# omarkhursheed/whisper-sae

Measured on AMD Instinct MI355X. Metric: activations/sec through SAE train step (d=384->3072, k=32), higher is better.
Workload: dtype bf16; 1 GPU; BASELINE.json configs[1]: TopKSAE 384->3072 k=32 train step, synthetic activations resident in the HBM ring buffer; batch_per_gpu=16384, global_batch=16384, ring_rows_per_gpu=4194304, parallelism=dp1

## Files before the change

whisper-sae_amd/csrc/wsae_common.h:

```cpp
#pragma once

#include <hip/hip_runtime.h>
#include <stdint.h>
#include <stdio.h>

#include "wsae.h"

void wsae_set_error(const char* fmt, ...);

#define WSAE_HIP_CHECK(expr)                                                              \
    do {                                                                                  \
        hipError_t e_ = (expr);                                                           \
        if (e_ != hipSuccess) {                                                           \
            wsae_set_error("%s failed: %s (%s:%d)", #expr, hipGetErrorString(e_), __FILE__, \
                           __LINE__);                                                     \
            return WSAE_ERR_HIP;                                                          \
        }                                                                                 \
    } while (0)

#define WSAE_REQUIRE(cond, ...)          \
    do {                                 \
        if (!(cond)) {                   \
            wsae_set_error(__VA_ARGS__); \
            return WSAE_ERR_INVALID;     \
        }                                \
    } while (0)

#define WSAE_LAUNCH_CHECK()                                                                  \
    do {                                                                                     \
        hipError_t e_ = hipGetLastError();                                                   \
        if (e_ != hipSuccess) {                                                              \
            wsae_set_error("kernel launch failed: %s (%s:%d)", hipGetErrorString(e_), __FILE__, \
                           __LINE__);                                                        \
            return WSAE_ERR_HIP;                                                             \
        }                                                                                    \
    } while (0)

typedef __bf16 bf16_t;
typedef __bf16 bf16x8 __attribute__((ext_vector_type(8)));
typedef __bf16 bf16x4 __attribute__((ext_vector_type(4)));
typedef float f32x16 __attribute__((ext_vector_type(16)));
typedef float f32x4 __attribute__((ext_vector_type(4)));
typedef float f32x2 __attribute__((ext_vector_type(2)));
typedef __bf16 bf16x2 __attribute__((ext_vector_type(2)));

static inline int64_t ceil_div64(int64_t a, int64_t b) { return (a + b - 1) / b; }
static inline int ceil_div(int a, int b) { return (a + b - 1) / b; }

#define WSAE_MAX_PARTIALS 1024
#define WSAE_WGRAD_MAX_SPLIT 8

struct wsae_prof {
    unsigned mask;
    int max_samples;
    int count[WSAE_K_COUNT];
    hipEvent_t* ev[WSAE_K_COUNT];
};

struct wsae_ctx {
    wsae_prof prof;
    int D, H, K, maxB, prec, device;
    const float* relu_l1w;
    int loss_cols;
    int cus;
    int comm_reserve;
    int64_t P;
    int64_t off[5];
    bf16_t* We_bf16;
    bf16_t* WdT_bf16;
    float* c_fold;
    void* xb;
    void* xT;
    void* gT;
    float* g;
    bf16_t* gb;
    int g_is_bf16;
    int xT_valid;
    int g32_valid;
    float* pre;
    float* smax;
    int smax_valid;
    uint32_t* tmin;
    int tmin_cur;
    int strip_predict;
    float tg_fixed_s;
    int pred_valid;
    const void* pred_x;
    const int32_t* pred_rows;
    float* part_loss;
    float* part_l0;
    float* part_dbd;
    float* part_sq;
    float* colnorm;
    float* wg_slabs;
    float* dbe_slab;
    float* dbpre_part;
    uint32_t* ent_pos;
    void* ent_hid;
    void* ent_dpre;
    int32_t* ent_off;
    int ent_valid;
    const float* ent_vals;
    int ent_B;
    const float* wire_dec_vals;
    int wire_dec_B;
    int32_t* counters;
    int32_t* dead_list;
    int32_t* row_order;
    int relu_fp8;
    void* relu_ws;
    int relu_x_B;
    int relu_g_B;
    float* fired;
    const float* wire_metrics;
    int n_dec_blocks;
    int n_sq_parts;
    float* dbd2;
    int32_t* btk_ws;
    int btk_k;
    int btk_mode;
    wsae_batch_topk_state* btk_state;
    size_t ws_bytes;
};

#define WSAE_PROF_BEGIN(ctx, id, st)                                                          \
    const bool prof_on_##id = ((ctx)->prof.mask >> (id)) & 1u &&                               \
                              (ctx)->prof.count[id] < (ctx)->prof.max_samples;                 \
    if (prof_on_##id) (void)hipEventRecord((ctx)->prof.ev[id][2 * (ctx)->prof.count[id]], st)
#define WSAE_PROF_END(ctx, id, st)                                                            \
    if (prof_on_##id) {                                                                       \
        (void)hipEventRecord((ctx)->prof.ev[id][2 * (ctx)->prof.count[id] + 1], st);           \
        (ctx)->prof.count[id]++;                                                              \
    }

#ifdef __HIPCC__

#define WSAE_WAVE 64

template <int M>
__device__ __forceinline__ uint32_t lane_xor_u32(uint32_t x, int lane) {
    if constexpr (M == 1) return (uint32_t)__builtin_amdgcn_update_dpp(0, (int)x, 0xB1, 0xF, 0xF, false);
    else if constexpr (M == 2) return (uint32_t)__builtin_amdgcn_update_dpp(0, (int)x, 0x4E, 0xF, 0xF, false);
    else if constexpr (M == 4) {
        const uint32_t up = (uint32_t)__builtin_amdgcn_update_dpp(0, (int)x, 0x104, 0xF, 0xF, false);
        const uint32_t dn = (uint32_t)__builtin_amdgcn_update_dpp(0, (int)x, 0x114, 0xF, 0xF, false);
        return (lane & 4) ? dn : up;
    } else if constexpr (M == 8) return (uint32_t)__builtin_amdgcn_update_dpp(0, (int)x, 0x128, 0xF, 0xF, false);
    else if constexpr (M == 16) {
        const auto r = __builtin_amdgcn_permlane16_swap((int)x, (int)x, false, false);
        return (uint32_t)((lane & 16) ? r[0] : r[1]);
    } else {
        static_assert(M == 32, "lane_xor_u32: M must be a power of two <= 32");
        const auto r = __builtin_amdgcn_permlane32_swap((int)x, (int)x, false, false);
        return (uint32_t)((lane & 32) ? r[0] : r[1]);
    }
}

__device__ __forceinline__ float wave_sum(float v) {
    const int lane = threadIdx.x & 63;
    v += __uint_as_float(lane_xor_u32<32>(__float_as_uint(v), lane));
    v += __uint_as_float(lane_xor_u32<16>(__float_as_uint(v), lane));
    v += __uint_as_float(lane_xor_u32<8>(__float_as_uint(v), lane));
    v += __uint_as_float(lane_xor_u32<4>(__float_as_uint(v), lane));
    v += __uint_as_float(lane_xor_u32<2>(__float_as_uint(v), lane));
    v += __uint_as_float(lane_xor_u32<1>(__float_as_uint(v), lane));
    return v;
}
__device__ __forceinline__ float wave_max(float v) {
    const int lane = threadIdx.x & 63;
    v = fmaxf(v, __uint_as_float(lane_xor_u32<32>(__float_as_uint(v), lane)));
    v = fmaxf(v, __uint_as_float(lane_xor_u32<16>(__float_as_uint(v), lane)));
    v = fmaxf(v, __uint_as_float(lane_xor_u32<8>(__float_as_uint(v), lane)));
    v = fmaxf(v, __uint_as_float(lane_xor_u32<4>(__float_as_uint(v), lane)));
    v = fmaxf(v, __uint_as_float(lane_xor_u32<2>(__float_as_uint(v), lane)));
    v = fmaxf(v, __uint_as_float(lane_xor_u32<1>(__float_as_uint(v), lane)));
    return v;
}
__device__ __forceinline__ int wave_sum_i(int v) {
    const int lane = threadIdx.x & 63;
    v += (int)lane_xor_u32<32>((uint32_t)v, lane);
    v += (int)lane_xor_u32<16>((uint32_t)v, lane);
    v += (int)lane_xor_u32<8>((uint32_t)v, lane);
    v += (int)lane_xor_u32<4>((uint32_t)v, lane);
    v += (int)lane_xor_u32<2>((uint32_t)v, lane);
    v += (int)lane_xor_u32<1>((uint32_t)v, lane);
    return v;
}

__device__ __forceinline__ float block_sum(float v, float* scratch) {
    v = wave_sum(v);
    const int lane = threadIdx.x & 63, w = threadIdx.x >> 6, nw = blockDim.x >> 6;
    __syncthreads();
    if (lane == 0) scratch[w] = v;
    __syncthreads();
    float r = 0.f;
    if (threadIdx.x == 0)
        for (int i = 0; i < nw; ++i) r += scratch[i];
    return r;
}

#define TICKET_GROUPS 32
#define TICKET_WORDS (1 + TICKET_GROUPS)
__device__ __forceinline__ bool grid_ticket(unsigned long long* t, unsigned payload, unsigned* total) {
    const unsigned nblk = gridDim.x * gridDim.y;
    const unsigned bid = blockIdx.y * gridDim.x + blockIdx.x;
    const unsigned ngrp = nblk < TICKET_GROUPS ? nblk : TICKET_GROUPS;
    const unsigned grp = bid % ngrp;
    const unsigned gsz = (nblk - grp + ngrp - 1) / ngrp;
    const unsigned long long add = (1ull << 32) | payload;
    const unsigned long long o1 = __hip_atomic_fetch_add(t + 1 + grp, add, __ATOMIC_RELAXED, __HIP_MEMORY_SCOPE_AGENT);
    if ((unsigned)(o1 >> 32) != gsz - 1) return false;
    __hip_atomic_store(t + 1 + grp, 0ull, __ATOMIC_RELAXED, __HIP_MEMORY_SCOPE_AGENT);
    const unsigned long long add2 = (1ull << 32) | (unsigned)((o1 + add) & 0xFFFFFFFFull);
    const unsigned long long o2 = __hip_atomic_fetch_add(t, add2, __ATOMIC_RELAXED, __HIP_MEMORY_SCOPE_AGENT);
    if ((unsigned)(o2 >> 32) != ngrp - 1) return false;
    __hip_atomic_store(t, 0ull, __ATOMIC_RELAXED, __HIP_MEMORY_SCOPE_AGENT);
    *total = (unsigned)((o2 + add2) & 0xFFFFFFFFull);
    return true;
}

__device__ __forceinline__ float4 nt_load4(const float4* p) {
    const f32x4 v = __builtin_nontemporal_load((const f32x4*)p);
    return make_float4(v[0], v[1], v[2], v[3]);
}
__device__ __forceinline__ void nt_store4(float4* p, const float4& a) {
    f32x4 v;
    v[0] = a.x; v[1] = a.y; v[2] = a.z; v[3] = a.w;
    __builtin_nontemporal_store(v, (f32x4*)p);
}

template <int DT>
__device__ __forceinline__ float load_act(const void* p, int64_t i) {
    if (DT == WSAE_DT_BF16) return (float)((const bf16_t*)p)[i];
    return ((const float*)p)[i];
}

#endif

int wsae_internal_stage(wsae_ctx* ctx, const float* params, const void* x, int x_dtype, const int32_t* rows, int B, hipStream_t st);
int wsae_internal_stage_rows(wsae_ctx* ctx, const float* params, const void* x, int x_dtype, const int32_t* rows, int B, hipStream_t st);
int wsae_internal_stage_and_gemm(wsae_ctx* ctx, const float* params, const void* x, int x_dtype, const int32_t* rows,
                                 int B, float* pre, int64_t* step_count, int direct, hipStream_t st, bool predicate = false);
int wsae_internal_topk(wsae_ctx* ctx, int B, float* vals, int32_t* idx, int32_t* fb, hipStream_t st);
int wsae_internal_encode_topk(wsae_ctx* ctx, const float* params, const void* x, int x_dtype, const int32_t* rows, int B,
                              float* vals, int32_t* idx, int64_t* step_count, int32_t* fb, hipStream_t st);
bool wsae_internal_strips_ok(const wsae_ctx* ctx);
size_t wsae_internal_batch_topk_ws_bytes();
int wsae_internal_batch_topk(wsae_ctx* ctx, float* vals, int B, int k_batch, int mode, wsae_batch_topk_state* state,
                             hipStream_t st);
bool wsae_internal_decode_mfma_ok(const wsae_ctx* c);
int wsae_internal_decode_mfma(wsae_ctx* c, const float* params, const void* x, int x_dtype, const int32_t* rows,
                              const float* vals, const int32_t* idx, int B, float* recon, int want_bwd, float* dpre,
                              int want_g32, int64_t* last_activated, const int64_t* step_count, wsae_stats* stats,
                              hipStream_t st);
bool wsae_internal_gemm256d_fp8(wsae_ctx* c, const void* A, int64_t lda, const void* Bt, int64_t ldb, const float* rscale,
                                const float* cscale, const float* bias, float* C, int64_t ldc, int M, int N, int K,
                                hipStream_t st);
bool wsae_internal_gemm256d(wsae_ctx* c, const void* A, int64_t lda, const void* Bt, int64_t ldb, const float* bias, float* C,
                            int64_t ldc, int M, int N, int K, int nsplit, int64_t cz, hipStream_t st);

enum { GX_EPI_PLAIN = 0, GX_EPI_RELU = 1, GX_EPI_DPRE = 2 };
struct GxEpi {
    const float* bias;
    float* c;
    int64_t ldc, cz;
    bf16_t* out16;
    uint64_t* bits;
    int64_t ldbits;
    int64_t ld16;
    const float* colw;
    float l1;
    float* part;
    int nslots;
    float* colpart;
    const float* rscale;
    const float* cscale;
    float* rowmax;
};
bool wsae_internal_gemm256x(wsae_ctx* c, int a_rm, int b_rm, int epi, const void* A, int64_t lda, const void* Bm, int64_t ldb,
                            int M, int N, int K, int nsplit, const GxEpi& e, hipStream_t st, int fp8 = 0);
int wsae_internal_relu_wgrad(wsae_ctx* ctx, const void* hid, const void* dpre, const void* xb, const void* gb, int B, float* grads,
                             hipStream_t st);
```

whisper-sae_amd/csrc/wsae_encode.hip:

```cpp
#include "wsae_common.h"
#include "wsae_mfma.h"
#include "wsae_topk.h"

template <typename T>
__device__ __forceinline__ void store4(T* p, const float (&v)[4]) {
    if (sizeof(T) == 2) {
        bf16x4 o;
#pragma unroll
        for (int i = 0; i < 4; ++i) o[i] = (bf16_t)v[i];
        *(bf16x4*)p = o;
    } else {
        *(float4*)p = make_float4(v[0], v[1], v[2], v[3]);
    }
}

template <int XDT>
__device__ __forceinline__ void load4(const void* x, int64_t i, float (&v)[4]) {
    if (XDT == WSAE_DT_BF16) {
        const bf16x4 t = *(const bf16x4*)((const bf16_t*)x + i);
#pragma unroll
        for (int q = 0; q < 4; ++q) v[q] = (float)t[q];
    } else {
        const float4 t = *(const float4*)((const float*)x + i);
        v[0] = t.x; v[1] = t.y; v[2] = t.z; v[3] = t.w;
// ... 263 lines not shown
                        const float rs = rscale[min(b, B - 1)];
                        v.x *= rs * cs4.x; v.y *= rs * cs4.y; v.z *= rs * cs4.z; v.w *= rs * cs4.w;
                    }
                    v.x += bv4.x; v.y += bv4.y; v.z += bv4.z; v.w += bv4.w;
                    if (b < B && hcol < H) *(float4*)(Cz + (int64_t)b * ldp + hcol) = v;
                    if (smax) {
                        float m = fmaxf(fmaxf(v.x, v.y), fmaxf(v.z, v.w));
                        m = fmaxf(m, __int_as_float(__builtin_amdgcn_update_dpp(0, __float_as_int(m), 0xB1, 0xF, 0xF, false)));
                        m = fmaxf(m, __int_as_float(__builtin_amdgcn_update_dpp(0, __float_as_int(m), 0x4E, 0xF, 0xF, false)));
                        if ((lane & 3) == 0 && b < B && hcol < H) smax[(int64_t)b * (H >> 4) + (hcol >> 4)] = m;
                    }
                }
                __builtin_amdgcn_wave_barrier();
            }
        }
#pragma unroll
        for (int j = 0; j < 4; ++j) ar[j] = ar_n[j];
    }
    dma_wait();
#ifdef WSAE_ENC_STAMPS
    if (lane == 0)
        for (int i = 0; i < 8; ++i) atomicAdd(&enc_stamp_sum[i], en_acc[i]);
#endif
}
template <typename T>
__device__ __forceinline__ void slab_load_rows(SlabRegs<T>& r, const T* __restrict__ base, int64_t ld, const int32_t* __restrict__ arows,
                                               int row0, int n_rows, int k0, int k_total, int tid) {
    constexpr int EPC = 16 / (int)sizeof(T);
    auto chunk = [&](int c) -> uint4 {
        const int row = row0 + (c >> 3), k = k0 + (c & 7) * EPC;
        if (row < n_rows && k < k_total) return *(const uint4*)(base + (int64_t)arows[row] * ld + k);
        return make_uint4(0, 0, 0, 0);
    };
    r.v0 = chunk(tid); r.v1 = chunk(tid + 256); r.v2 = chunk(tid + 512); r.v3 = chunk(tid + 768);
}

template <typename T>
__global__ void __launch_bounds__(256)
encode_gemm_kernel(const T* __restrict__ xb, const T* __restrict__ W, const float* __restrict__ bias,
                   float* __restrict__ pre, int ldp, int B, int H, int D, const int32_t* __restrict__ arows,
                   int64_t* __restrict__ step_count) {
    extern __shared__ __attribute__((aligned(16))) char smem[];
    char* As = smem;
    char* Bs = smem + TILE_LDS_BYTES;
    const int tid = threadIdx.x, lane = tid & 63, wave = tid >> 6;
    const int wm = wave >> 1, wn = wave & 1;
    const int m0 = blockIdx.y * TILE_M, n0 = blockIdx.x * TILE_N;
    constexpr int KT = Mfma<T>::KT;
    if (step_count && blockIdx.x == 0 && blockIdx.y == 0 && tid == 0) *step_count += 1;

    f32x16 acc[2][2];
#pragma unroll
    for (int i = 0; i < 2; ++i)
#pragma unroll
        for (int j = 0; j < 2; ++j)
#pragma unroll
            for (int r = 0; r < 16; ++r) acc[i][j][r] = 0.f;

    SlabRegs<T> ra, rb;
    if (arows) slab_load_rows<T>(ra, xb, D, arows, m0, B, 0, D, tid);
    else slab_load<T>(ra, xb, D, m0, B, 0, D, tid);
    slab_load<T>(rb, W, D, n0, H, 0, D, tid);
    const int nk = (D + KT - 1) / KT;
    for (int kt = 0; kt < nk; ++kt) {
        slab_store<T>(ra, As, tid);
        slab_store<T>(rb, Bs, tid);
        __syncthreads();
        if (kt + 1 < nk) {
            if (arows) slab_load_rows<T>(ra, xb, D, arows, m0, B, (kt + 1) * KT, D, tid);
            else slab_load<T>(ra, xb, D, m0, B, (kt + 1) * KT, D, tid);
            slab_load<T>(rb, W, D, n0, H, (kt + 1) * KT, D, tid);
        }
        Mfma<T>::slab(As, Bs, wm * 64, wn * 64, lane, acc);
        __syncthreads();
    }
    const int col = lane & 31, rq = lane >> 5;
#pragma unroll
    for (int mi = 0; mi < 2; ++mi)
#pragma unroll
        for (int ni = 0; ni < 2; ++ni) {
            const int h = n0 + wn * 64 + ni * 32 + col;
            if (h >= H) continue;
            const float bv = bias[h];
#pragma unroll
            for (int r = 0; r < 16; ++r) {
                const int b = m0 + wm * 64 + mi * 32 + (r & 3) + 8 * (r >> 2) + 4 * rq;
                if (b < B) pre[(int64_t)b * ldp + h] = acc[mi][ni][r] + bv;
            }
        }
}

__global__ void __launch_bounds__(256)
encode_direct_kernel(const bf16_t* __restrict__ xa, const int32_t* __restrict__ arows, const bf16_t* __restrict__ W,
                     const float* __restrict__ bias, float* __restrict__ pre, int ldp, int B, int H, int D,
                     int64_t* __restrict__ step_count) {
    const int lane = threadIdx.x & 63, wave = threadIdx.x >> 6;
    if (step_count && blockIdx.x == 0 && blockIdx.y == 0 && threadIdx.x == 0) *step_count += 1;
    const int n0 = blockIdx.x * 32, m0 = blockIdx.y * 128 + wave * 32;
    if (m0 >= B) return;
    const int r = lane & 31, h = lane >> 5;
    const int mrow = min(m0 + r, B - 1);
    const int64_t arow = arows ? (int64_t)arows[mrow] : (int64_t)mrow;
    const bf16_t* ap = xa + arow * D + 8 * h;
    const bf16_t* bp = W + (int64_t)min(n0 + r, H - 1) * D + 8 * h;
    f32x16 acc;
#pragma unroll
    for (int i = 0; i < 16; ++i) acc[i] = 0.f;
    const int nk = D / 16;
    for (int k0 = 0; k0 < nk; k0 += 8) {
        bf16x8 a[8], b[8];
#pragma unroll
        for (int j = 0; j < 8; ++j) {
            const int kk = min(k0 + j, nk - 1);
            a[j] = *(const bf16x8*)(ap + 16 * kk);
            b[j] = *(const bf16x8*)(bp + 16 * kk);
        }
#pragma unroll
        for (int j = 0; j < 8; ++j)
            if (k0 + j < nk) acc = __builtin_amdgcn_mfma_f32_32x32x16_bf16(a[j], b[j], acc, 0, 0, 0);
    }
    const int n = n0 + r;
    if (n >= H) return;
    const float bv = bias[n];
#pragma unroll
    for (int i = 0; i < 16; ++i) {
        const int m = m0 + (i & 3) + 8 * (i >> 2) + 4 * h;
        if (m < B) pre[(int64_t)m * ldp + n] = acc[i] + bv;
    }
}

#define TOPK_CAP 256

__global__ void __launch_bounds__(256) topk_kernel(const float* __restrict__ pre, int B, int H, int K,
                                                   float* __restrict__ vals, int32_t* __restrict__ idx,
                                                   int32_t* __restrict__ fallback_rows) {
    __shared__ uint64_t lists[4][TOPK_CAP];
    const int lane = threadIdx.x & 63, wave = threadIdx.x >> 6;
    const int b = blockIdx.x * 4 + wave;
    if (b >= B) return;
    const float* row = pre + (int64_t)b * H;
    uint64_t* list = lists[wave];
    float* vrow = vals + (int64_t)b * K;
    int32_t* irow = idx + (int64_t)b * K;

    uint64_t kmin = 0;
    if (K <= 64) {
        float m = -INFINITY;
        bool any = false;
        for (int e = lane * 4; e < H; e += 256) {
            const float4 v = *(const float4*)(row + e);
            m = fmaxf(fmaxf(m, fmaxf(v.x, v.y)), fmaxf(v.z, v.w));
            any = true;
        }
        uint64_t mk[1] = {any ? ((uint64_t)f32_ord(m) << 32) : 0ull};
        wave_sort_desc<1>(mk, lane);
        const uint32_t thi = __shfl((uint32_t)(mk[0] >> 32), K - 1, 64);
        kmin = (uint64_t)thi << 32;
    }
    const int count = topk_compact<TOPK_CAP>(row, H, kmin, list, lane);
    if (count > TOPK_CAP || count < K) {
        topk_row_generic<TOPK_CAP>(row, H, K, list, lane, vrow, irow, fallback_rows);
        return;
    }
    topk_emit_any<TOPK_CAP>(list, count, K, lane, vrow, irow);
}

#define TOPK_STRIP 8

template <int VPL>
__global__ void __launch_bounds__(256)
topk_rows_kernel(const float* __restrict__ pre, int B, int H, int K, float* __restrict__ vals,
                 int32_t* __restrict__ idx, int32_t* __restrict__ fallback_rows) {
    __shared__ uint64_t lists[4][TOPK_CAP];
    __shared__ uint64_t strips[4][64 * TOPK_STRIP];
    const int lane = threadIdx.x & 63, wave = threadIdx.x >> 6;
    const int b = blockIdx.x * 4 + wave;
    if (b >= B) return;
    const float* row = pre + (int64_t)b * H;
    uint64_t* list = lists[wave];
    uint64_t* strip = strips[wave] + lane * TOPK_STRIP;

    float4 v[VPL];
    float m = -INFINITY;
#pragma unroll
    for (int i = 0; i < VPL; ++i) {
        const int e = lane * 4 + 256 * i;
        v[i] = e < H ? *(const float4*)(row + e) : make_float4(-INFINITY, -INFINITY, -INFINITY, -INFINITY);
        m = fmaxf(fmaxf(m, fmaxf(v[i].x, v[i].y)), fmaxf(v[i].z, v[i].w));
    }
    uint32_t mk[1] = {f32_ord(m)};
    wave_sort_desc<1, uint32_t>(mk, lane);
    const uint32_t thi = __shfl(mk[0], K - 1, 64);

    int cnt = 0;
#pragma unroll
    for (int i = 0; i < VPL; ++i) {
        const float vv[4] = {v[i].x, v[i].y, v[i].z, v[i].w};
#pragma unroll
        for (int c = 0; c < 4; ++c) {
            const uint32_t o = f32_ord(vv[c]);
            if (o >= thi && lane * 4 + 256 * i + c < H) {
                if (cnt < TOPK_STRIP) strip[cnt] = ((uint64_t)o << 32) | (uint32_t)(~(uint32_t)(lane * 4 + 256 * i + c));
                ++cnt;
            }
        }
    }
    int incl = cnt;
#pragma unroll
    for (int o = 1; o < 64; o <<= 1) {
        const int n = __shfl_up(incl, o, 64);
        if (lane >= o) incl += n;
    }
    const int total = __shfl(incl, 63, 64);
    float* vrow = vals + (int64_t)b * K;
    int32_t* irow = idx + (int64_t)b * K;
    if (__any(cnt > TOPK_STRIP) || total > TOPK_CAP || total < K) {
        topk_row_generic<TOPK_CAP>(row, H, K, list, lane, vrow, irow, fallback_rows);
        return;
    }
    const int off = incl - cnt;
    for (int s_ = 0; s_ < cnt; ++s_) list[off + s_] = strip[s_];
    __builtin_amdgcn_wave_barrier();
    topk_emit_any<TOPK_CAP>(list, total, K, lane, vrow, irow);
}

template <int SPL, int NTOP>
__global__ void __launch_bounds__(256) __attribute__((amdgpu_waves_per_eu(8, 8)))
topk_strips_kernel(const float* pre, const float* __restrict__ smax, int B, int H, int K,
                   float* __restrict__ vals, int32_t* __restrict__ idx, int32_t* __restrict__ fallback_rows, StripFix fix,
                   const uint32_t* tmin) {
    __shared__ uint64_t lists[4][TOPK_CAP];
    __shared__ int strips[4][TS_MAX_STRIPS];
    const int lane = threadIdx.x & 63, wave = threadIdx.x >> 6;
    const int b = blockIdx.x * 4 + wave;
    if (b >= B) return;
    fix.tg = tmin ? *(const float*)(tmin + TG_USED) : -INFINITY;
    topk_strips_row<SPL, NTOP, TOPK_CAP>(pre + (int64_t)b * H, smax + (int64_t)b * (H >> 4), H, K, lane, lists[wave],
                                         strips[wave], vals + (int64_t)b * K, idx + (int64_t)b * K, fallback_rows, nullptr,
                                         nullptr, tmin != nullptr, fix, b);
}

__global__ void __launch_bounds__(256) densify_kernel(const float* __restrict__ vals, const int32_t* __restrict__ idx,
                                                      int B, int H, int K, float* __restrict__ hidden) {
    const int64_t i = (int64_t)blockIdx.x * 256 + threadIdx.x;
    if (i >= (int64_t)B * K) return;
    const int b = (int)(i / K);
    const float v = vals[i];
    hidden[(int64_t)b * H + idx[i]] = v > 0.f ? v : 0.f;
}

static int round_up(int a, int b) { return (a + b - 1) / b * b; }

template <typename T>
static int stage_batch(wsae_ctx* c, const float* params, const void* x, int x_dtype, const int32_t* rows, int B,
                       int64_t* step_count, hipStream_t st, bool want_xT = true) {
    const int D = c->D;
    const int ldT = round_up(B, 128);
    dim3 sg(ceil_div(ldT, 64), ceil_div(D, 64));
    T* xT = want_xT ? (T*)c->xT : nullptr;
    WSAE_PROF_BEGIN(c, WSAE_K_STAGE_BATCH, st);
    if (!want_xT && sizeof(T) == 2 && x_dtype == WSAE_DT_BF16 && D % 8 == 0) {
        const int64_t nchunks = (int64_t)B * (D / 8);
        stage_rows_copy_kernel<<<(unsigned)ceil_div64(nchunks, 512), 256, 0, st>>>((const uint4*)x, rows, (uint4*)c->xb, nchunks, D / 8,
                                                                                 step_count);
    } else if (x_dtype == WSAE_DT_F32)
        stage_batch_kernel<WSAE_DT_F32, T><<<sg, 256, 0, st>>>(x, rows, params + c->off[4], (T*)c->xb, xT, B, D, ldT, step_count);
    else
        stage_batch_kernel<WSAE_DT_BF16, T><<<sg, 256, 0, st>>>(x, rows, params + c->off[4], (T*)c->xb, xT, B, D, ldT, step_count);
    WSAE_PROF_END(c, WSAE_K_STAGE_BATCH, st);
    WSAE_LAUNCH_CHECK();
    return WSAE_OK;
}

template <typename T>
static bool persistent_ok(const wsae_ctx* c, int B) {
    constexpr int KT = SWZ_ROW_BYTES / (int)sizeof(T);
    return B >= 2048 && c->H % 256 == 0 && c->D % (2 * KT) == 0;
}

template <typename T>
static int gemm_dense(wsae_ctx* c, const float* params, int B, float* pre, int ldp, const T* xa, const int32_t* arows,
                      int64_t* step_count, hipStream_t st, bool predicate = false) {
    const T* W = sizeof(T) == 2 ? (const T*)c->We_bf16 : (const T*)(params + c->off[0]);
    const float* bias = sizeof(T) == 2 ? c->c_fold : params + c->off[2];
    const int H = c->H;
    WSAE_PROF_BEGIN(c, WSAE_K_ENCODE_GEMM, st);
    if (persistent_ok<T>(c, B)) {
        const int ntn = H / 256, ntiles = ntn * ceil_div(B, 256);
        float* smax = (pre == c->pre && ldp == H) ? c->smax : nullptr;
        uint32_t* tmin = nullptr;
        if (pre == c->pre) c->pred_valid = 0;
        if (predicate && smax && sizeof(T) == 2) {
            c->tmin_cur = (c->tmin_cur + 1) % 3;
            tmin = c->tmin;
            c->pred_valid = 1;
            c->pred_x = xa;
            c->pred_rows = arows;
        }
        encode_gemm256d_kernel<T><<<min(ntiles, c->cus), 512, G256D_LDS, st>>>(xa, c->D, W, c->D, bias, pre, ldp, B, H, c->D, ntn,
                                                                              ntiles, 1, 0, smax, arows, step_count, nullptr,
                                                                              nullptr, tmin, c->tmin_cur, c->tg_fixed_s);
        if (pre == c->pre) c->smax_valid = smax ? 1 : 0;
    } else if (sizeof(T) == 2 && B <= 1024 && c->D % 16 == 0) {
        if (pre == c->pre) c->smax_valid = c->pred_valid = 0;
        encode_direct_kernel<<<dim3(ceil_div(H, 32), ceil_div(B, 128)), 256, 0, st>>>((const bf16_t*)xa, arows, (const bf16_t*)W, bias, pre,
                                                                                     ldp, B, H, c->D, step_count);
    } else {
        if (pre == c->pre) c->smax_valid = c->pred_valid = 0;
        dim3 gg(ceil_div(H, TILE_N), ceil_div(B, TILE_M));
        encode_gemm_kernel<T><<<gg, 256, 2 * TILE_LDS_BYTES, st>>>(xa, W, bias, pre, ldp, B, H, c->D, arows, step_count);
    }
    WSAE_PROF_END(c, WSAE_K_ENCODE_GEMM, st);
    WSAE_LAUNCH_CHECK();
    return WSAE_OK;
}

template <typename T>
static int stage_and_gemm(wsae_ctx* c, const float* params, const void* x, int x_dtype, const int32_t* rows, int B,
                          float* pre, int64_t* step_count, int direct, hipStream_t st, bool predicate = false) {
    if (direct && sizeof(T) == 2 && x_dtype == WSAE_DT_BF16) {
        c->xT_valid = 0;
        return gemm_dense<T>(c, params, B, pre, c->H, (const T*)x, rows, step_count, st, predicate);
    }
    int rc = stage_batch<T>(c, params, x, x_dtype, rows, B, step_count, st);
    if (rc) return rc;
    c->xT_valid = 1;
    return gemm_dense<T>(c, params, B, pre, c->H, (const T*)c->xb, nullptr, nullptr, st, predicate);
}

static int check_batch(const wsae_ctx* c, const void* x, int x_dtype, int B, const char* who) {
    WSAE_REQUIRE(c && x, "%s: null argument", who);
    WSAE_REQUIRE(B >= 1 && B <= c->maxB, "%s: batch %d outside [1, max_batch=%d]", who, B, c->maxB);
    WSAE_REQUIRE(x_dtype == WSAE_DT_F32 || x_dtype == WSAE_DT_BF16, "%s: unknown activation dtype %d", who, x_dtype);
    return WSAE_OK;
}

template <typename T>
static bool gemm256d_try(wsae_ctx* c, const void* A, int64_t lda, const void* Bt, int64_t ldb, const float* bias, float* C,
                         int64_t ldc, int M, int N, int K, int nsplit, int64_t cz, hipStream_t st) {
    constexpr int KT = SWZ_ROW_BYTES / (int)sizeof(T);
    if (M < 512 || N < 128 || N % 4 || K % nsplit || (K / nsplit) % (2 * KT) || lda % (16 / (int)sizeof(T)) ||
        ldb % (16 / (int)sizeof(T)) || ldc % 4)
        return false;
    const int ntn = ceil_div(N, 256), ntiles_mn = ntn * ceil_div(M, 256);
    encode_gemm256d_kernel<T><<<min(ntiles_mn * nsplit, c->cus), 512, G256D_LDS, st>>>((const T*)A, lda, (const T*)Bt, ldb, bias, C, ldc,
// ... 132 lines not shown
```

whisper-sae_amd/csrc/wsae_topk.h:

```cpp
#pragma once

#include "wsae_common.h"

__device__ __forceinline__ uint32_t f32_ord(float f) {
    const uint32_t u = __float_as_uint(f);
    return (u & 0x80000000u) ? ~u : (u | 0x80000000u);
}
__device__ __forceinline__ float ord_f32(uint32_t o) {
    return __uint_as_float((o & 0x80000000u) ? (o & 0x7FFFFFFFu) : ~o);
}
template <int M>
__device__ __forceinline__ uint64_t lane_xor_u64(uint64_t v, int lane) {
    return ((uint64_t)lane_xor_u32<M>((uint32_t)(v >> 32), lane) << 32) | lane_xor_u32<M>((uint32_t)v, lane);
}

template <int M>
__device__ __forceinline__ uint64_t lane_xor_key(uint64_t k, int lane) { return lane_xor_u64<M>(k, lane); }
template <int M>
__device__ __forceinline__ uint32_t lane_xor_key(uint32_t k, int lane) { return lane_xor_u32<M>(k, lane); }

template <int NPL, typename KT>
__device__ __forceinline__ KT xor_partner(KT k, int stride, int lane) {
    switch (stride / NPL) {
        case 1: return lane_xor_key<1>(k, lane);
        case 2: return lane_xor_key<2>(k, lane);
        case 4: return lane_xor_key<4>(k, lane);
        case 8: return lane_xor_key<8>(k, lane);
        case 16: return lane_xor_key<16>(k, lane);
        default: return lane_xor_key<32>(k, lane);
    }
}

template <int NPL, typename KT = uint64_t>
__device__ __forceinline__ void wave_sort_desc(KT (&key)[NPL], int lane) {
#pragma unroll
    for (int size = 2; size <= 64 * NPL; size <<= 1) {
#pragma unroll
        for (int stride = size >> 1; stride > 0; stride >>= 1) {
            if (stride >= NPL) {
#pragma unroll
                for (int i = 0; i < NPL; ++i) {
                    const KT other = xor_partner<NPL>(key[i], stride, lane);
                    const int p = lane * NPL + i;
                    const bool desc = (p & size) == 0;
                    const bool lower = (p & stride) == 0;
                    const bool keep_max = (lower == desc);
                    key[i] = ((key[i] > other) == keep_max) ? key[i] : other;
                }
            } else {
#pragma unroll
                for (int i = 0; i < NPL; ++i) {
                    if ((i & stride) == 0) {
                        const int j = i | stride;
                        const int p = lane * NPL + i;
                        const bool desc = (p & size) == 0;
                        const KT a = key[i], b = key[j];
                        const bool swap = (a > b) != desc;
                        key[i] = swap ? b : a;
                        key[j] = swap ? a : b;
                    }
                }
            }
        }
    }
}

template <int NPL>
__device__ __forceinline__ void topk_emit(const uint64_t* list, int count, int K, int lane, float* vrow, int32_t* irow,
                                          float* vs = nullptr, int32_t* is = nullptr) {
    uint64_t key[NPL];
#pragma unroll
    for (int i = 0; i < NPL; ++i) {
        const int p = lane * NPL + i;
        key[i] = p < count ? list[p] : 0ull;
    }
    wave_sort_desc<NPL>(key, lane);
#pragma unroll
    for (int i = 0; i < NPL; ++i) {
        const int p = lane * NPL + i;
        if (p < K) {
            const float v = ord_f32((uint32_t)(key[i] >> 32));
            const int32_t f = (int32_t)(~(uint32_t)key[i]);
            vrow[p] = v;
            irow[p] = f;
            if (vs) {
                vs[p] = v;
                is[p] = f;
            }
        }
    }
}

template <int CAP>
__device__ __forceinline__ void topk_emit_any(const uint64_t* list, int count, int K, int lane, float* vrow,
                                              int32_t* irow, float* vs = nullptr, int32_t* is = nullptr) {
    if (count <= 64) topk_emit<1>(list, count, K, lane, vrow, irow, vs, is);
    else if (CAP <= 128 || count <= 128) topk_emit<2>(list, count, K, lane, vrow, irow, vs, is);
    else topk_emit<4>(list, count, K, lane, vrow, irow, vs, is);
}

template <int CAP>
__device__ __forceinline__ int topk_compact(const float* __restrict__ row, int H, uint64_t kmin, uint64_t* list,
                                            int lane) {
    int base = 0;
    for (int e0 = 0; e0 < H; e0 += 256) {
        const int e = e0 + lane * 4;
        float4 v = make_float4(0, 0, 0, 0);
        const bool in = e < H;
        if (in) v = *(const float4*)(row + e);
        const float vv[4] = {v.x, v.y, v.z, v.w};
#pragma unroll
        for (int c = 0; c < 4; ++c) {
            const uint64_t key = ((uint64_t)f32_ord(vv[c]) << 32) | (uint32_t)(~(uint32_t)(e + c));
            const bool pass = in && key >= kmin;
            const unsigned long long m = __ballot(pass);
            if (m) {
                const int pos = base + __popcll(m & ((1ull << lane) - 1ull));
                if (pass && pos < CAP) list[pos] = key;
                base += __popcll(m);
            }
        }
    }
    return base;
}

__device__ __forceinline__ int topk_count_ge(const float* __restrict__ row, int H, uint64_t kmin, int lane) {
    int cnt = 0;
    for (int e0 = 0; e0 < H; e0 += 256) {
        const int e = e0 + lane * 4;
        if (e < H) {
            const float4 v = *(const float4*)(row + e);
            const float vv[4] = {v.x, v.y, v.z, v.w};
#pragma unroll
            for (int c = 0; c < 4; ++c) {
                const uint64_t key = ((uint64_t)f32_ord(vv[c]) << 32) | (uint32_t)(~(uint32_t)(e + c));
                cnt += key >= kmin ? 1 : 0;
            }
        }
    }
    return wave_sum_i(cnt);
}

template <int CAP>
__device__ __noinline__ void topk_row_generic(const float* row, int H, int K, uint64_t* list, int lane, float* vrow,
                                              int32_t* irow, int32_t* fallback_rows, float* vs = nullptr,
                                              int32_t* is = nullptr) {
    if (lane == 0) atomicAdd(fallback_rows, 1);
    uint64_t prefix = 0;
    for (int bit = 63; bit >= 0; --bit) {
        const uint64_t cand = prefix | (1ull << bit);
        if (topk_count_ge(row, H, cand, lane) >= K) prefix = cand;
    }
    const int count = topk_compact<CAP>(row, H, prefix, list, lane);
    if (count <= 64) topk_emit<1>(list, count, K, lane, vrow, irow, vs, is);
    else topk_emit<2>(list, count, K, lane, vrow, irow, vs, is);
}

#define TS_MAX_STRIPS 128

#define TG_S_START 0.95f
#define TG_S_MAX 1.0f
#define TG_S_MIN 0.25f
#define TG_S_DOWN 0.9f
#define TG_S_UP 0.005f

#define TG_SLOTS 64
#define TG_SLOT_STRIDE 64
#define TG_GROUP_WORDS (TG_SLOTS * TG_SLOT_STRIDE)
#define TG_HDR_S 1
#define TG_HDR_MISSES 2
#define TG_USED (3 * TG_GROUP_WORDS)
#define TG_REFILLED (3 * TG_GROUP_WORDS + 1)
#define TG_WORDS (3 * TG_GROUP_WORDS + 16)

__device__ __forceinline__ float strip_store_threshold(const uint32_t* slots, int cur, int lane, float fixed_s, float* s_out) {
    const uint32_t* prev = slots + ((cur + 2) % 3) * TG_GROUP_WORDS;
    const uint32_t* prev2 = slots + ((cur + 1) % 3) * TG_GROUP_WORDS;
    uint32_t a = __builtin_nontemporal_load(prev + lane * TG_SLOT_STRIDE);
    uint32_t b = __builtin_nontemporal_load(prev2 + lane * TG_SLOT_STRIDE);
    const float s_prev = __uint_as_float(__builtin_nontemporal_load(prev + TG_HDR_S));
    const int misses = (int)__builtin_nontemporal_load(prev + TG_HDR_MISSES);
    float s = !(s_prev > 0.f) ? TG_S_START : misses > 0 ? fmaxf(s_prev * TG_S_DOWN, TG_S_MIN) : fminf(s_prev + TG_S_UP, TG_S_MAX);
    if (fixed_s > 0.f) s = fixed_s;
    *s_out = s;
    if (a == 0u) a = 0xFFFFFFFFu;
    if (b == 0u) b = 0xFFFFFFFFu;
    uint32_t o = a < b ? a : b;
    o = min(o, lane_xor_u32<1>(o, lane));
    o = min(o, lane_xor_u32<2>(o, lane));
    o = min(o, lane_xor_u32<4>(o, lane));
    o = min(o, lane_xor_u32<8>(o, lane));
    o = min(o, lane_xor_u32<16>(o, lane));
    o = min(o, lane_xor_u32<32>(o, lane));
    o = (uint32_t)__builtin_amdgcn_readfirstlane((int)o);
    if (o == 0xFFFFFFFFu) return -INFINITY;
    const float t = ord_f32(o);
    return t > 0.f ? s * t : -INFINITY;
}

struct StripFix {
    const bf16_t* x;
    const int32_t* arows;
    const bf16_t* We;
    const float* bias;
    int D;
    float tg;
    uint32_t* tmin_group;
    int32_t* miss_rows;
};

__device__ __forceinline__ void strip_fix_note(const StripFix& f, uint32_t thi, int b, int lane) {
    if (f.tmin_group && (b & 3) == 0 && lane == 0) atomicMin(f.tmin_group + ((b >> 2) & (TG_SLOTS - 1)) * TG_SLOT_STRIDE, thi);
}

typedef const __attribute__((address_space(1))) bf16x8* gptr_bf16x8;
typedef __attribute__((address_space(3))) char* lds_bytes;

template <bool XS>
__device__ __noinline__ void strip_fix_fill(const bf16_t* xrow, const bf16_t* We, const float* bias, int D, int32_t* miss_rows,
                                            int32_t* group_misses, const int* masks, int nwords, lds_bytes xs, float* prow, int lane) {
    if (lane == 0) {
        atomicAdd(miss_rows, 1);
        atomicAdd(group_misses, 1);
    }
    const int r = lane & 31, h = lane >> 5;
    gptr_bf16x8 ap = (gptr_bf16x8)(uintptr_t)(xrow + 8 * h);
    if constexpr (XS) {
        for (int c = lane; c < (D >> 3); c += 64) *(__attribute__((address_space(3))) bf16x8*)(xs + 16 * c) = *(gptr_bf16x8)(uintptr_t)(xrow + 8 * c);
        __builtin_amdgcn_wave_barrier();
    }
    constexpr int NB = XS ? 8 : 4;
    for (int w = 0; w < nwords; ++w) {
        const uint32_t m = (uint32_t)__builtin_amdgcn_readfirstlane(masks[w]);
        uint32_t pairs = (m | (m >> 1)) & 0x55555555u;
        while (pairs) {
            const int p = __builtin_ctz(pairs);
            pairs &= pairs - 1;
            const int blk = (32 * w + p) >> 1;
            const bool n0 = (m >> p) & 1u, n1 = (m >> (p + 1)) & 1u;
            gptr_bf16x8 bp = (gptr_bf16x8)(uintptr_t)(We + (int64_t)(blk * 32 + r) * D + 8 * h);
            f32x16 acc;
#pragma unroll
            for (int i = 0; i < 16; ++i) acc[i] = 0.f;
            for (int s0 = 0; s0 < (D >> 4); s0 += NB) {
                bf16x8 bv[NB], av[XS ? 1 : NB];
#pragma unroll
                for (int j = 0; j < NB; ++j) {
                    bv[j] = bp[2 * (s0 + j)];
                    if constexpr (!XS) av[j] = ap[2 * (s0 + j)];
                }
#pragma unroll
                for (int j = 0; j < NB; ++j) {
                    if constexpr (XS) av[0] = *(const __attribute__((address_space(3))) bf16x8*)(xs + 32 * (s0 + j) + 16 * h);
                    acc = __builtin_amdgcn_mfma_f32_32x32x16_bf16(av[XS ? 0 : j], bv[j], acc, 0, 0, 0);
                }
            }
            const float v = acc[0] + bias[blk * 32 + r];
            if (h == 0 && (r < 16 ? n0 : n1)) prow[blk * 32 + r] = v;
        }
    }
    __threadfence();
}

template <int SPL, int CAP>
__device__ __forceinline__ int strips_collect(const float* row, const float (&sm)[SPL], int ns, uint32_t th, int lane,
                                              uint64_t* list, int* slist) {
    int nstr = 0;
#pragma unroll
    for (int i = 0; i < SPL; ++i) {
        const bool pass = lane + 64 * i < ns && f32_ord(sm[i]) >= th;
        const unsigned long long mask = __ballot(pass);
        const int pos = nstr + __popcll(mask & ((1ull << lane) - 1ull));
        if (pass && pos < TS_MAX_STRIPS) slist[pos] = lane + 64 * i;
        nstr += __popcll(mask);
    }
    if (nstr > TS_MAX_STRIPS) return -1;
    __builtin_amdgcn_wave_barrier();
    int total = 0;
    for (int base = 0; base < nstr; base += 16) {
        const int si = base + (lane >> 2);
        const bool in = si < nstr;
        const int s = in ? slist[si] : 0;
        const int e = s * 16 + (lane & 3) * 4;
        float4 v = make_float4(0.f, 0.f, 0.f, 0.f);
        if (in) v = nt_load4((const float4*)(row + e));
        const float vv[4] = {v.x, v.y, v.z, v.w};
#pragma unroll
        for (int c = 0; c < 4; ++c) {
            const uint32_t o = f32_ord(vv[c]);
            const bool pass = in && o >= th;
            const unsigned long long mask = __ballot(pass);
            if (mask) {
                const int pos = total + __popcll(mask & ((1ull << lane) - 1ull));
                if (pass && pos < CAP) list[pos] = ((uint64_t)o << 32) | (uint32_t)(~(uint32_t)(e + c));
                total += __popcll(mask);
            }
        }
    }
    __builtin_amdgcn_wave_barrier();
    return total;
}

template <int SPL, int CAP>
__device__ __forceinline__ void strips_refill(const StripFix& fix, int b, const float (&sm)[SPL], int ns, uint32_t lo, int lane,
                                              uint64_t* list, int* slist, float* row) {
    if (!(fix.tg > -INFINITY)) return;
#pragma unroll
    for (int i = 0; i < SPL; ++i) {
        const bool want = lane + 64 * i < ns && sm[i] < fix.tg && f32_ord(sm[i]) >= lo;
        const unsigned long long m = __ballot(want);
        if (lane == 0) {
            slist[2 * i] = (int)(uint32_t)m;
            slist[2 * i + 1] = (int)(uint32_t)(m >> 32);
        }
    }
    __builtin_amdgcn_wave_barrier();
    const bf16_t* xrow = fix.x + (int64_t)(fix.arows ? fix.arows[b] : b) * fix.D;
    if (fix.D <= 4 * CAP)
        strip_fix_fill<true>(xrow, fix.We, fix.bias, fix.D, fix.miss_rows, (int32_t*)fix.tmin_group + TG_HDR_MISSES, slist, 2 * SPL, (lds_bytes)(char*)list, row, lane);
    else
        strip_fix_fill<false>(xrow, fix.We, fix.bias, fix.D, fix.miss_rows, (int32_t*)fix.tmin_group + TG_HDR_MISSES, slist, 2 * SPL, nullptr, row, lane);
    __builtin_amdgcn_wave_barrier();
}

template <int SPL, int CAP>
__device__ __noinline__ void topk_strips_row_rare(const float* row, const float* srow, int H, int K, int lane, uint64_t* list,
                                                  int* slist, float* vrow, int32_t* irow, int32_t* fallback_rows, float* vs,
                                                  int32_t* is, StripFix fix, int b, uint32_t thi, int full) {
    const int ns = H >> 4;
    float sm[SPL];
#pragma unroll
    for (int i = 0; i < SPL; ++i) sm[i] = lane + 64 * i < ns ? srow[lane + 64 * i] : -INFINITY;
    if (!full) {
        int total = strips_collect<SPL, CAP>(row, sm, ns, f32_ord(fix.tg), lane, list, slist);
        if (total >= 0 && total < K) {
            strips_refill<SPL, CAP>(fix, b, sm, ns, thi, lane, list, slist, (float*)row);
            total = strips_collect<SPL, CAP>(row, sm, ns, thi, lane, list, slist);
        }
        if (total >= K && total <= CAP) {
            topk_emit_any<CAP>(list, total, K, lane, vrow, irow, vs, is);
            return;
        }
    }
    strips_refill<SPL, CAP>(fix, b, sm, ns, 0u, lane, list, slist, (float*)row);
    topk_row_generic<CAP>(row, H, K, list, lane, vrow, irow, fallback_rows, vs, is);
}

template <int SPL, int NTOP, int CAP>
__device__ __forceinline__ void topk_strips_row(const float* row, const float* __restrict__ srow, int H,
                                                int K, int lane, uint64_t* list, int* slist, float* vrow,
                                                int32_t* irow, int32_t* fallback_rows, float* vs = nullptr,
                                                int32_t* is = nullptr, bool pred = false, const StripFix& fix = StripFix(), int b = 0) {
    const int ns = H >> 4;
    float sm[SPL];
    float m = -INFINITY, m2 = -INFINITY;
#pragma unroll
    for (int i = 0; i < SPL; ++i) {
        const int s = lane + 64 * i;
        sm[i] = s < ns ? __builtin_nontemporal_load(srow + s) : -INFINITY;
        m2 = fmaxf(m2, fminf(m, sm[i]));
        m = fmaxf(m, sm[i]);
    }
    uint32_t thi;
    if constexpr (NTOP == 1) {
        uint32_t mk[1] = {f32_ord(m)};
        wave_sort_desc<1, uint32_t>(mk, lane);
        thi = (uint32_t)__builtin_amdgcn_readlane((int)mk[0], K - 1);
    } else {
        uint32_t mk[2] = {f32_ord(m), f32_ord(m2)};
        wave_sort_desc<2, uint32_t>(mk, lane);
        const uint32_t lo = (uint32_t)__builtin_amdgcn_readlane((int)mk[0], (K - 1) >> 1);
        const uint32_t hi = (uint32_t)__builtin_amdgcn_readlane((int)mk[1], (K - 1) >> 1);
        thi = ((K - 1) & 1) ? hi : lo;
    }
    if (pred) {
        strip_fix_note(fix, thi, b, lane);
        if (!(ord_f32(thi) >= fix.tg)) {
            topk_strips_row_rare<SPL, CAP>(row, srow, H, K, lane, list, slist, vrow, irow, fallback_rows, vs, is, fix, b, thi, 0);
            return;
        }
    }
    const int total = strips_collect<SPL, CAP>(row, sm, ns, thi, lane, list, slist);
    if (total < 0 || total > CAP || total < K) {
        if (pred) topk_strips_row_rare<SPL, CAP>(row, srow, H, K, lane, list, slist, vrow, irow, fallback_rows, vs, is, fix, b, thi, 1);
        else topk_row_generic<CAP>(row, H, K, list, lane, vrow, irow, fallback_rows, vs, is);
        return;
    }
    topk_emit_any<CAP>(list, total, K, lane, vrow, irow, vs, is);
}
```

Before: 72.55 million activations/s.

## Replace wave bitonic threshold sort with ballot radix select and prefetch strip loads

```diff
diff --git a/whisper-sae_amd/csrc/wsae_common.h b/whisper-sae_amd/csrc/wsae_common.h
--- a/whisper-sae_amd/csrc/wsae_common.h
+++ b/whisper-sae_amd/csrc/wsae_common.h
@@ -139,20 +139,20 @@
 
 template <int M>
 __device__ __forceinline__ uint32_t lane_xor_u32(uint32_t x, int lane) {
-    if constexpr (M == 1) return (uint32_t)__builtin_amdgcn_update_dpp(0, (int)x, 0xB1, 0xF, 0xF, false);
-    else if constexpr (M == 2) return (uint32_t)__builtin_amdgcn_update_dpp(0, (int)x, 0x4E, 0xF, 0xF, false);
+    (void)lane;
+    if constexpr (M == 1) return (uint32_t)__builtin_amdgcn_mov_dpp((int)x, 0xB1, 0xF, 0xF, true);
+    else if constexpr (M == 2) return (uint32_t)__builtin_amdgcn_mov_dpp((int)x, 0x4E, 0xF, 0xF, true);
     else if constexpr (M == 4) {
-        const uint32_t up = (uint32_t)__builtin_amdgcn_update_dpp(0, (int)x, 0x104, 0xF, 0xF, false);
-        const uint32_t dn = (uint32_t)__builtin_amdgcn_update_dpp(0, (int)x, 0x114, 0xF, 0xF, false);
-        return (lane & 4) ? dn : up;
-    } else if constexpr (M == 8) return (uint32_t)__builtin_amdgcn_update_dpp(0, (int)x, 0x128, 0xF, 0xF, false);
+        const int up = __builtin_amdgcn_mov_dpp((int)x, 0x104, 0xF, 0x5, false);
+        return (uint32_t)__builtin_amdgcn_update_dpp(up, (int)x, 0x114, 0xF, 0xA, false);
+    } else if constexpr (M == 8) return (uint32_t)__builtin_amdgcn_mov_dpp((int)x, 0x128, 0xF, 0xF, true);
     else if constexpr (M == 16) {
         const auto r = __builtin_amdgcn_permlane16_swap((int)x, (int)x, false, false);
-        return (uint32_t)((lane & 16) ? r[0] : r[1]);
+        return (uint32_t)(__builtin_amdgcn_inverse_ballot_w64(0xFFFF0000FFFF0000ull) ? r[0] : r[1]);
     } else {
         static_assert(M == 32, "lane_xor_u32: M must be a power of two <= 32");
         const auto r = __builtin_amdgcn_permlane32_swap((int)x, (int)x, false, false);
-        return (uint32_t)((lane & 32) ? r[0] : r[1]);
+        return (uint32_t)(__builtin_amdgcn_inverse_ballot_w64(0xFFFFFFFF00000000ull) ? r[0] : r[1]);
     }
 }
 
diff --git a/whisper-sae_amd/csrc/wsae_encode.hip b/whisper-sae_amd/csrc/wsae_encode.hip
--- a/whisper-sae_amd/csrc/wsae_encode.hip
+++ b/whisper-sae_amd/csrc/wsae_encode.hip
@@ -439,9 +439,8 @@
             m = fmaxf(fmaxf(m, fmaxf(v.x, v.y)), fmaxf(v.z, v.w));
             any = true;
         }
-        uint64_t mk[1] = {any ? ((uint64_t)f32_ord(m) << 32) : 0ull};
-        wave_sort_desc<1>(mk, lane);
-        const uint32_t thi = __shfl((uint32_t)(mk[0] >> 32), K - 1, 64);
+        const uint32_t mk[1] = {any ? f32_ord(m) : 0u};
+        const uint32_t thi = wave_kth_largest<1>(mk, K);
         kmin = (uint64_t)thi << 32;
     }
     const int count = topk_compact<TOPK_CAP>(row, H, kmin, list, lane);
@@ -475,9 +474,8 @@
         v[i] = e < H ? *(const float4*)(row + e) : make_float4(-INFINITY, -INFINITY, -INFINITY, -INFINITY);
         m = fmaxf(fmaxf(m, fmaxf(v[i].x, v[i].y)), fmaxf(v[i].z, v[i].w));
     }
-    uint32_t mk[1] = {f32_ord(m)};
-    wave_sort_desc<1, uint32_t>(mk, lane);
-    const uint32_t thi = __shfl(mk[0], K - 1, 64);
+    const uint32_t mk[1] = {f32_ord(m)};
+    const uint32_t thi = wave_kth_largest<1>(mk, K);
 
     int cnt = 0;
 #pragma unroll
diff --git a/whisper-sae_amd/csrc/wsae_topk.h b/whisper-sae_amd/csrc/wsae_topk.h
--- a/whisper-sae_amd/csrc/wsae_topk.h
+++ b/whisper-sae_amd/csrc/wsae_topk.h
@@ -4,7 +4,7 @@
 
 __device__ __forceinline__ uint32_t f32_ord(float f) {
     const uint32_t u = __float_as_uint(f);
-    return (u & 0x80000000u) ? ~u : (u | 0x80000000u);
+    return u ^ ((uint32_t)((int32_t)u >> 31) | 0x80000000u);
 }
 __device__ __forceinline__ float ord_f32(uint32_t o) {
     return __uint_as_float((o & 0x80000000u) ? (o & 0x7FFFFFFFu) : ~o);
@@ -14,55 +14,68 @@
     return ((uint64_t)lane_xor_u32<M>((uint32_t)(v >> 32), lane) << 32) | lane_xor_u32<M>((uint32_t)v, lane);
 }
 
-template <int M>
-__device__ __forceinline__ uint64_t lane_xor_key(uint64_t k, int lane) { return lane_xor_u64<M>(k, lane); }
-template <int M>
-__device__ __forceinline__ uint32_t lane_xor_key(uint32_t k, int lane) { return lane_xor_u32<M>(k, lane); }
-
-template <int NPL, typename KT>
-__device__ __forceinline__ KT xor_partner(KT k, int stride, int lane) {
-    switch (stride / NPL) {
-        case 1: return lane_xor_key<1>(k, lane);
-        case 2: return lane_xor_key<2>(k, lane);
-        case 4: return lane_xor_key<4>(k, lane);
-        case 8: return lane_xor_key<8>(k, lane);
-        case 16: return lane_xor_key<16>(k, lane);
-        default: return lane_xor_key<32>(k, lane);
-    }
-}
-
-template <int NPL, typename KT = uint64_t>
-__device__ __forceinline__ void wave_sort_desc(KT (&key)[NPL], int lane) {
-#pragma unroll
-    for (int size = 2; size <= 64 * NPL; size <<= 1) {
-#pragma unroll
-        for (int stride = size >> 1; stride > 0; stride >>= 1) {
-            if (stride >= NPL) {
-#pragma unroll
-                for (int i = 0; i < NPL; ++i) {
-                    const KT other = xor_partner<NPL>(key[i], stride, lane);
-                    const int p = lane * NPL + i;
-                    const bool desc = (p & size) == 0;
-                    const bool lower = (p & stride) == 0;
-                    const bool keep_max = (lower == desc);
-                    key[i] = ((key[i] > other) == keep_max) ? key[i] : other;
-                }
+template <int N>
+__device__ __forceinline__ uint32_t wave_kth_largest(const uint32_t (&key)[N], int K) {
+    uint32_t prefix = 0;
+#pragma unroll
+    for (int bit = 31; bit >= 0; --bit) {
+        const uint32_t cand = prefix | (1u << bit);
+        int n = 0;
+#pragma unroll
+        for (int i = 0; i < N; ++i) n += __popcll(__builtin_amdgcn_ballot_w64(key[i] >= cand));
+        prefix = n >= K ? cand : prefix;
+    }
+    return prefix;
+}
+
+constexpr uint64_t sort_lane_mask(int npl, int size, int stride) {
+    uint64_t m = 0;
+    for (int l = 0; l < 64; ++l) {
+        const int p = l * npl;
+        if (((p & size) == 0) == ((p & stride) == 0)) m |= 1ull << l;
+    }
+    return m;
+}
+
+template <int NPL, int SIZE, int STRIDE>
+__device__ __forceinline__ void wave_sort_step(uint64_t (&key)[NPL], int lane) {
+    if constexpr (STRIDE >= NPL) {
+        const bool keep_max = __builtin_amdgcn_inverse_ballot_w64(sort_lane_mask(NPL, SIZE, STRIDE));
+#pragma unroll
+        for (int i = 0; i < NPL; ++i) {
+            constexpr int M = STRIDE / NPL;
+            if constexpr (M >= 16) {
+                const uint32_t hi = (uint32_t)(key[i] >> 32), lo = (uint32_t)key[i];
+                const auto rh = M == 16 ? __builtin_amdgcn_permlane16_swap(hi, hi, false, false) : __builtin_amdgcn_permlane32_swap(hi, hi, false, false);
+                const auto rl = M == 16 ? __builtin_amdgcn_permlane16_swap(lo, lo, false, false) : __builtin_amdgcn_permlane32_swap(lo, lo, false, false);
+                const uint64_t a = ((uint64_t)rh[0] << 32) | rl[0], b = ((uint64_t)rh[1] << 32) | rl[1];
+                key[i] = ((a > b) == keep_max) ? a : b;
             } else {
-#pragma unroll
-                for (int i = 0; i < NPL; ++i) {
-                    if ((i & stride) == 0) {
-                        const int j = i | stride;
-                        const int p = lane * NPL + i;
-                        const bool desc = (p & size) == 0;
-                        const KT a = key[i], b = key[j];
-                        const bool swap = (a > b) != desc;
-                        key[i] = swap ? b : a;
-                        key[j] = swap ? a : b;
-                    }
-                }
-            }
-        }
-    }
+                const uint64_t other = lane_xor_u64<M>(key[i], lane);
+                key[i] = ((key[i] > other) == keep_max) ? key[i] : other;
+            }
+        }
+    } else {
+        const bool desc_lane = SIZE >= NPL ? __builtin_amdgcn_inverse_ballot_w64(sort_lane_mask(NPL, SIZE, 0)) : false;
+#pragma unroll
+        for (int i = 0; i < NPL; ++i) {
+            if ((i & STRIDE) == 0) {
+                const int j = i | STRIDE;
+                const bool desc = SIZE >= NPL ? desc_lane : (i & SIZE) == 0;
+                const uint64_t a = key[i], b = key[j];
+                const bool swap = (a > b) != desc;
+                key[i] = swap ? b : a;
+                key[j] = swap ? a : b;
+            }
+        }
+    }
+    if constexpr (STRIDE > 1) wave_sort_step<NPL, SIZE, STRIDE / 2>(key, lane);
+}
+
+template <int NPL, int SIZE = 2>
+__device__ __forceinline__ void wave_sort_desc(uint64_t (&key)[NPL], int lane) {
+    wave_sort_step<NPL, SIZE, SIZE / 2>(key, lane);
+    if constexpr (SIZE < 64 * NPL) wave_sort_desc<NPL, SIZE * 2>(key, lane);
 }
 
 template <int NPL>
@@ -262,6 +275,28 @@
     __threadfence();
 }
 
+__device__ __forceinline__ int lanes_below(unsigned long long mask, int base) {
+    return (int)__builtin_amdgcn_mbcnt_hi((uint32_t)(mask >> 32), __builtin_amdgcn_mbcnt_lo((uint32_t)mask, (uint32_t)base));
+}
+
+template <int CAP>
+__device__ __forceinline__ int strips_file(const float4 v, bool in, int e, uint32_t th, int total, uint64_t* list, int bound) {
+    const float vv[4] = {v.x, v.y, v.z, v.w};
+    const uint32_t ne = ~(uint32_t)e;
+    const unsigned long long inmask = __builtin_amdgcn_ballot_w64(in);
+#pragma unroll
+    for (int c = 0; c < 4; ++c) {
+        const uint32_t o = f32_ord(vv[c]);
+        const bool pass = in && o >= th;
+        const unsigned long long mask = __builtin_amdgcn_ballot_w64(o >= th) & inmask;
+        const int pos = lanes_below(mask, total);
+        if (pass && (bound <= CAP || pos < CAP)) list[pos] = ((uint64_t)o << 32) | (ne - (uint32_t)c);
+        total += __popcll(mask);
+    }
+    return total;
+}
+
+#define TS_AHEAD 3
 template <int SPL, int CAP>
 __device__ __forceinline__ int strips_collect(const float* row, const float (&sm)[SPL], int ns, uint32_t th, int lane,
                                               uint64_t* list, int* slist) {
@@ -269,33 +304,34 @@
 #pragma unroll
     for (int i = 0; i < SPL; ++i) {
         const bool pass = lane + 64 * i < ns && f32_ord(sm[i]) >= th;
-        const unsigned long long mask = __ballot(pass);
-        const int pos = nstr + __popcll(mask & ((1ull << lane) - 1ull));
+        const unsigned long long mask = __builtin_amdgcn_ballot_w64(f32_ord(sm[i]) >= th) & __builtin_amdgcn_ballot_w64(lane + 64 * i < ns);
+        const int pos = lanes_below(mask, nstr);
         if (pass && pos < TS_MAX_STRIPS) slist[pos] = lane + 64 * i;
         nstr += __popcll(mask);
     }
     if (nstr > TS_MAX_STRIPS) return -1;
     __builtin_amdgcn_wave_barrier();
+    const int sub = lane >> 2, col = (lane & 3) * 4;
+    float4 v[TS_AHEAD];
+    int e[TS_AHEAD];
+#pragma unroll
+    for (int j = 0; j < TS_AHEAD; ++j) {
+        const int si = 16 * j + sub;
+        e[j] = (si < nstr ? slist[si] : 0) * 16 + col;
+        v[j] = make_float4(0.f, 0.f, 0.f, 0.f);
+        if (si < nstr) v[j] = nt_load4((const float4*)(row + e[j]));
+    }
     int total = 0;
-    for (int base = 0; base < nstr; base += 16) {
-        const int si = base + (lane >> 2);
+#pragma unroll
+    for (int j = 0; j < TS_AHEAD; ++j)
+        if (16 * j < nstr) total = strips_file<CAP>(v[j], 16 * j + sub < nstr, e[j], th, total, list, 256 * (j + 1));
+    for (int base = 16 * TS_AHEAD; base < nstr; base += 16) {
+        const int si = base + sub;
         const bool in = si < nstr;
-        const int s = in ? slist[si] : 0;
-        const int e = s * 16 + (lane & 3) * 4;
-        float4 v = make_float4(0.f, 0.f, 0.f, 0.f);
-        if (in) v = nt_load4((const float4*)(row + e));
-        const float vv[4] = {v.x, v.y, v.z, v.w};
-#pragma unroll
-        for (int c = 0; c < 4; ++c) {
-            const uint32_t o = f32_ord(vv[c]);
-            const bool pass = in && o >= th;
-            const unsigned long long mask = __ballot(pass);
-            if (mask) {
-                const int pos = total + __popcll(mask & ((1ull << lane) - 1ull));
-                if (pass && pos < CAP) list[pos] = ((uint64_t)o << 32) | (uint32_t)(~(uint32_t)(e + c));
-                total += __popcll(mask);
-            }
-        }
+        const int ee = (in ? slist[si] : 0) * 16 + col;
+        float4 w = make_float4(0.f, 0.f, 0.f, 0.f);
+        if (in) w = nt_load4((const float4*)(row + ee));
+        total = strips_file<CAP>(w, in, ee, th, total, list, 16 * TS_MAX_STRIPS);
     }
     __builtin_amdgcn_wave_barrier();
     return total;
@@ -363,15 +399,11 @@
     }
     uint32_t thi;
     if constexpr (NTOP == 1) {
-        uint32_t mk[1] = {f32_ord(m)};
-        wave_sort_desc<1, uint32_t>(mk, lane);
-        thi = (uint32_t)__builtin_amdgcn_readlane((int)mk[0], K - 1);
+        const uint32_t mk[1] = {f32_ord(m)};
+        thi = wave_kth_largest<1>(mk, K);
     } else {
-        uint32_t mk[2] = {f32_ord(m), f32_ord(m2)};
-        wave_sort_desc<2, uint32_t>(mk, lane);
-        const uint32_t lo = (uint32_t)__builtin_amdgcn_readlane((int)mk[0], (K - 1) >> 1);
-        const uint32_t hi = (uint32_t)__builtin_amdgcn_readlane((int)mk[1], (K - 1) >> 1);
-        thi = ((K - 1) & 1) ? hi : lo;
+        const uint32_t mk[2] = {f32_ord(m), f32_ord(m2)};
+        thi = wave_kth_largest<2>(mk, K);
     }
     if (pred) {
         strip_fix_note(fix, thi, b, lane);
```

New measurement: 72.55 million activations/s, median of 3. Within noise of the previous version (-0.0%).
